# thomasneff/AdaNeRF

Measured on AMD Instinct MI355X. Metric: FPS at 800x800, higher is better.
Workload: dtype bf16

## Files before the change

adanerf_amd/csrc/k_mlp16.hip.hpp:

```cpp
#pragma once
#include "k_common.hip.hpp"
#include "k_mlp_f32.hip.hpp"
#include "tuning.hpp"
#include <utility>

namespace adanerf {


struct ShadeArgs {
  ShadeParams sp;
  NetParams net;
  const float* rays;
  const uint32_t* sample_key;
  const float* sample_z;
  const int32_t* total;
  int32_t max_samples;
  float* raw_out;
};

__device__ __forceinline__ void store_raw(const ShadeArgs& a, int s, float r, float g, float b, float alpha) {
  const float ks = a.net.out_scale[1];
  *reinterpret_cast<float4*>(a.raw_out + static_cast<size_t>(s) * 4) = make_float4(r * ks, g * ks, b * ks, alpha * a.net.out_scale[0]);
}

struct Bf16 {
  static constexpr bool kClampRelu = true;
  typedef bf16x8 vec8;
  static __device__ __forceinline__ uint32_t pack(float lo, float hi) {
    f32x2 v = {lo, hi};
    return __builtin_bit_cast(uint32_t, __builtin_convertvector(v, bf16x2));
  }
  static __device__ __forceinline__ f32x16 mfma(u32x4 a, u32x4 b, f32x16 c) {
    return __builtin_amdgcn_mfma_f32_32x32x16_bf16(__builtin_bit_cast(bf16x8, a), __builtin_bit_cast(bf16x8, b), c, 0, 0, 0);
  }
};
struct Fp16 {
  static constexpr bool kClampRelu = false;
  typedef f16x8 vec8;
  static __device__ __forceinline__ uint32_t pack(float lo, float hi) {
    f32x2 v = {lo, hi};
    return __builtin_bit_cast(uint32_t, __builtin_convertvector(v, f16x2));
  }
  static __device__ __forceinline__ f32x16 mfma(u32x4 a, u32x4 b, f32x16 c) {
    return __builtin_amdgcn_mfma_f32_32x32x16_f16(__builtin_bit_cast(f16x8, a), __builtin_bit_cast(f16x8, b), c, 0, 0, 0);
  }
};

using tune::kRegFrags;
constexpr int kShadeFrags16 = 32 + 4 * 128 + 160 + 2 * 128 + 144 + 72 + 8;
constexpr int kShadeBiasFloats = 8 * 256 + 288 + 128 + 32;

template <int CF, int RS, int LPW, int NR = kRegFrags>
struct WStream {
  static constexpr int kRegs = NR;
  static constexpr int kChunk = CF;
  static constexpr int kChunkBytes = CF * 1024;
#if defined(__HIP_DEVICE_COMPILE__)
  __amdgpu_buffer_rsrc_t rsrc;
#endif
  const char* gbase;
  uint32_t gbytes;
  uint32_t goff;
  uint32_t lane_off;
  uint32_t wave_off;
  uint32_t slot_cur;
  uint32_t rd_cur;
  uint32_t rd_next;
  uint32_t lds_base;
  uint32_t grp;
  uint32_t issuer;
  uint32_t dma_lds;
  uint32_t dma_goff;
  bool stag;
  u32x4 R[NR];
};

__device__ __forceinline__ u32x4 lds_read128(uint32_t byte_addr) {
  typedef const __attribute__((address_space(3))) u32x4* lds_u32x4_ptr;
  return *((lds_u32x4_ptr)(uintptr_t)byte_addr);
}

template <int CF, int RS, int LPW, int NR>
__device__ __forceinline__ void ws_piece(WStream<CF, RS, LPW, NR>& st, int i) {
  static_assert(LPW >= 1 && LPW <= 8, "a piece is addressed by the 12-bit immediate offset of buffer_load ... lds (pieces 4 .. 7: a second base)");
#if defined(__HIP_DEVICE_COMPILE__)
  typedef __attribute__((address_space(3))) void* lds_ptr;
  const uint32_t far = i >= 4 ? 4096u : 0u;
  lds_ptr dst = (lds_ptr) static_cast<uintptr_t>(st.dma_lds + far);
  const int voff = static_cast<int>(st.lane_off), soff = static_cast<int>(st.dma_goff + far);
  if (tune::kAblateDmaBytes) {
    if ((i & 3) == 0) __builtin_amdgcn_raw_ptr_buffer_load_lds(st.rsrc, dst, 4, voff, soff, 0, 0);
    else if ((i & 3) == 1) __builtin_amdgcn_raw_ptr_buffer_load_lds(st.rsrc, dst, 4, voff, soff, 1024, 0);
    else if ((i & 3) == 2) __builtin_amdgcn_raw_ptr_buffer_load_lds(st.rsrc, dst, 4, voff, soff, 2048, 0);
    else __builtin_amdgcn_raw_ptr_buffer_load_lds(st.rsrc, dst, 4, voff, soff, 3072, 0);
    return;
  }
  if ((i & 3) == 0) __builtin_amdgcn_raw_ptr_buffer_load_lds(st.rsrc, dst, 16, voff, soff, 0, 0);
  else if ((i & 3) == 1) __builtin_amdgcn_raw_ptr_buffer_load_lds(st.rsrc, dst, 16, voff, soff, 1024, 0);
  else if ((i & 3) == 2) __builtin_amdgcn_raw_ptr_buffer_load_lds(st.rsrc, dst, 16, voff, soff, 2048, 0);
  else __builtin_amdgcn_raw_ptr_buffer_load_lds(st.rsrc, dst, 16, voff, soff, 3072, 0);
#endif
}

template <int CF, int RS, int LPW, int NR>
__device__ __forceinline__ void ws_chunk_begin(WStream<CF, RS, LPW, NR>& st, uint32_t slot) {
  st.dma_lds = st.lds_base + slot * (CF * 1024) + st.wave_off;
  st.dma_goff = st.goff + st.wave_off;
  st.goff += CF * 1024;
  if (st.goff >= st.gbytes) st.goff = 0;
}

template <int CF, int RS, int LPW, int NR>
__device__ __forceinline__ void ws_issue(WStream<CF, RS, LPW, NR>& st, uint32_t slot) {
  ws_chunk_begin(st, slot);
#pragma unroll
  for (int i = 0; i < LPW; ++i) ws_piece(st, i);
}

__device__ __forceinline__ void ws_skip_pad() {
  if (tune::kSkipPad >= 0) asm volatile("s_nop %0" ::"n"(tune::kSkipPad < 0 ? 0 : tune::kSkipPad) : "memory");
}

template <int ABL, int CF, int RS, int LPW, int NR>
__device__ __forceinline__ void ws_sync(WStream<CF, RS, LPW, NR>& st, bool pad, int piece) {
  static_assert(RS >= 3 && (RS - 2) * LPW < 64, "vmcnt is a 6-bit counter");
  if (ABL & 1) return;
  if (!(ABL & 32)) asm volatile("s_waitcnt vmcnt(%0)\n\ts_barrier" ::"n"((RS - 3) * LPW) : "memory");
  const uint32_t slot = (st.grp == 0) ? st.slot_cur : (st.slot_cur == 0 ? RS - 1 : st.slot_cur - 1);
  if (!(ABL & 16)) {
    if (st.issuer) {
      ws_chunk_begin(st, slot);
      ws_piece(st, piece);
    } else if (pad) ws_skip_pad();
  }
}

template <int CF, int RS, int LPW, int NR>
__device__ __forceinline__ void ws_advance(WStream<CF, RS, LPW, NR>& st) {
  st.slot_cur = (st.slot_cur + 1 == RS) ? 0 : st.slot_cur + 1;
  const uint32_t nxt = (st.slot_cur + 1 == RS) ? 0 : st.slot_cur + 1;
  st.rd_cur = st.rd_next;
  st.rd_next = st.lds_base + nxt * (CF * 1024) + st.lane_off;
}


template <int ABL, int CF, int RS, int LPW, int NR>
__device__ __forceinline__ void ws_position(WStream<CF, RS, LPW, NR>& st, int f, bool tile_start) {
  constexpr int STEP = RS == 3 ? CF / LPW / 2 : CF / LPW;
  static_assert(CF % LPW == 0 && STEP >= 1 && (RS == 3 || (CF / 2) % STEP == 0), "piece positions: both groups' synchronisation points are piece positions");
  const bool pad = tile_start;
  const bool piece_pos = f % STEP == 0 && f / STEP < LPW && !(ABL & (1 | 16));
  if (f == 0) {
    if (ABL & 1) return;
    if (st.grp == 0) ws_sync<ABL>(st, pad, 0);
    else {
      if (pad) ws_skip_pad();
      if (piece_pos && st.issuer) ws_piece(st, 0);
    }
    ws_advance(st);
  } else if (f == CF / 2 && st.stag) {
    if (st.grp != 0) ws_sync<ABL>(st, pad, (CF / 2) / STEP);
    else {
      if (pad) ws_skip_pad();
      if (piece_pos && st.issuer) ws_piece(st, (CF / 2) / STEP);
    }
  } else if (piece_pos) {
    if (st.issuer) ws_piece(st, f / STEP);
  }
}

template <int ABL, int CF, int RS, int LPW, int NR>
__device__ __forceinline__ void ws_refill(WStream<CF, RS, LPW, NR>& st, int p) {
  if (ABL & 2) {
    asm volatile("" : "+v"(st.R[p % NR]));
    return;
  }
  const int q = p + NR;
  st.R[p % NR] = (q < CF) ? lds_read128(st.rd_cur + q * 1024) : lds_read128(st.rd_next + (q - CF) * 1024);
}

template <int CF, int RS, int LPW, int NR>
__device__ __forceinline__ void ws_start(WStream<CF, RS, LPW, NR>& st, const void* gbase, uint32_t gbytes, char* lds, int wave, int lane,
                                         int grp = -1, bool issuer = true) {
  st.stag = grp >= 0;
  st.grp = grp > 0 ? 1u : 0u;
  st.issuer = issuer;
  st.gbase = reinterpret_cast<const char*>(gbase);
  st.gbytes = gbytes;
#if defined(__HIP_DEVICE_COMPILE__)
  st.rsrc = __builtin_amdgcn_make_buffer_rsrc(const_cast<void*>(gbase), 0, static_cast<int>(gbytes), 0x00020000);
#endif
  st.goff = 0;
  st.lane_off = lane * 16;
  st.wave_off = wave * LPW * 1024;
  st.lds_base = static_cast<uint32_t>(reinterpret_cast<uintptr_t>(lds));
  if (issuer) {
#pragma unroll
    for (int k = 0; k < RS - 1; ++k) ws_issue(st, k);
  }
  asm volatile("s_waitcnt vmcnt(%0)\n\ts_barrier" ::"n"((RS - 2) * LPW) : "memory");
  st.slot_cur = RS - 1;
  st.rd_cur = st.lds_base + st.lane_off;
  st.rd_next = st.lds_base + st.lane_off;
#pragma unroll
  for (int i = 0; i < NR; ++i) st.R[i] = lds_read128(st.rd_next + i * 1024);
}

__device__ __forceinline__ float relu_keep_nan(float x) { return __builtin_elementwise_maximum(x, 0.0f); }

template <class ET, int F>
__device__ __forceinline__ void pe_pack(const float x[3], int h, uint32_t* out) {
  float t[pe_slots(F)];
  pe_eval<F, false>(x, h, t);
#pragma unroll
  for (int q = 0; q < pe_slots(F) / 2; ++q) out[q] = ET::pack(t[2 * q], t[2 * q + 1]);
}

struct BiasRegs {
  f32x4 b0, b1, b2, b3;
};
__device__ __forceinline__ void lds_bias_issue(uint32_t byte_addr, BiasRegs& r) {
  asm volatile("ds_read_b128 %0, %4\n\tds_read_b128 %1, %4 offset:16\n\tds_read_b128 %2, %4 offset:32\n\tds_read_b128 %3, %4 offset:48"
               : "=&v"(r.b0), "=&v"(r.b1), "=&v"(r.b2), "=&v"(r.b3)
               : "v"(byte_addr));
}
__device__ __forceinline__ void lds_bias_issue(uint32_t byte_addr, BiasRegs& r, uint32_t& rd0, uint32_t& rd1) {
  asm volatile("ds_read_b128 %0, %6\n\tds_read_b128 %1, %6 offset:16\n\tds_read_b128 %2, %6 offset:32\n\tds_read_b128 %3, %6 offset:48"
               : "=&v"(r.b0), "=&v"(r.b1), "=&v"(r.b2), "=&v"(r.b3), "+v"(rd0), "+v"(rd1)
               : "v"(byte_addr));
}
template <int YOUNGER = 0>
__device__ __forceinline__ void lds_bias_take(BiasRegs& r, f32x16* acc) {
  asm volatile("s_waitcnt lgkmcnt(%4)" : "+v"(r.b0), "+v"(r.b1), "+v"(r.b2), "+v"(r.b3) : "n"(YOUNGER > 15 ? 15 : YOUNGER));
  f32x16 a;
#pragma unroll
  for (int e = 0; e < 4; ++e) {
    a[e] = r.b0[e];
    a[4 + e] = r.b1[e];
    a[8 + e] = r.b2[e];
    a[12 + e] = r.b3[e];
  }
  *acc = a;
}

__device__ __forceinline__ void lds_bias16(uint32_t byte_addr, f32x16* acc) {
  f32x4 b0, b1, b2, b3;
  asm volatile("ds_read_b128 %0, %4\n\tds_read_b128 %1, %4 offset:16\n\tds_read_b128 %2, %4 offset:32\n\tds_read_b128 %3, %4 offset:48"
               : "=&v"(b0), "=&v"(b1), "=&v"(b2), "=&v"(b3)
               : "v"(byte_addr));
  asm volatile("s_waitcnt lgkmcnt(0)" : "+v"(b0), "+v"(b1), "+v"(b2), "+v"(b3));
  f32x16 a;
#pragma unroll
  for (int e = 0; e < 4; ++e) {
    a[e] = b0[e];
    a[4 + e] = b1[e];
    a[8 + e] = b2[e];
    a[12 + e] = b3[e];
  }
  *acc = a;
}

template <class ET, bool RELU>
__device__ __forceinline__ int mfma_guard(const f32x16& acc) {
  if constexpr (RELU && ET::kClampRelu) return __builtin_amdgcn_readfirstlane(__builtin_bit_cast(int, acc[15]));
  else return 0;
}

template <class ET, bool RELU>
__device__ __forceinline__ void epilogue_quad_16(const f32x16& acc, int m, int g, uint32_t* out, int guard = 0) {
  if constexpr (RELU && ET::kClampRelu) {
    uint32_t q0, q1;
    asm("v_cvt_pk_bf16_f32 %0, %1, %2 clamp\n\t; after the accumulator's guard %3" : "=v"(q0) : "v"(acc[4 * g + 0]), "v"(acc[4 * g + 1]), "s"(guard));
    asm("v_cvt_pk_bf16_f32 %0, %1, %2 clamp\n\t; after the accumulator's guard %3" : "=v"(q1) : "v"(acc[4 * g + 2]), "v"(acc[4 * g + 3]), "s"(guard));
    out[8 * m + 2 * g + 0] = q0;
    out[8 * m + 2 * g + 1] = q1;
    return;
  }
  uint32_t p0 = ET::pack(acc[4 * g + 0], acc[4 * g + 1]), p1 = ET::pack(acc[4 * g + 2], acc[4 * g + 3]);
  if (RELU) {
    if constexpr (std::is_same_v<ET, Fp16>) {
      const f16x2 z = {static_cast<_Float16>(0.f), static_cast<_Float16>(0.f)};
      p0 = __builtin_bit_cast(uint32_t, __builtin_elementwise_maximum(__builtin_bit_cast(f16x2, p0), z));
      p1 = __builtin_bit_cast(uint32_t, __builtin_elementwise_maximum(__builtin_bit_cast(f16x2, p1), z));
    } else {
      const s16x2 z = {0, 0};
      p0 = __builtin_bit_cast(uint32_t, __builtin_elementwise_max(__builtin_bit_cast(s16x2, p0), z));
      p1 = __builtin_bit_cast(uint32_t, __builtin_elementwise_max(__builtin_bit_cast(s16x2, p1), z));
    }
  }
  out[8 * m + 2 * g + 0] = p0;
  out[8 * m + 2 * g + 1] = p1;
}

constexpr int kKeepAllF32 = -2;


template <class ET, class WS, int S1, int S2, int MT, bool RELU, int FPOS, int KEEP_F32_TILE = -1>
__device__ __forceinline__ void layer_16(WS& st, uint32_t bias_addr, int lane, const uint32_t* in1, const uint32_t* in2,
                                         uint32_t* out, f32x16* keep = nullptr) {
  constexpr int CF = WS::kChunk;
  constexpr int KS = S1 + S2;
#pragma unroll
  for (int m = 0; m < MT; ++m) {
    f32x16 acc;
    if (tune::kAblateShade & 4) {
#pragma unroll
      for (int r = 0; r < 16; ++r) acc[r] = 0.f;
    } else {
      lds_bias16(bias_addr + m * 128, &acc);
    }
#pragma unroll
    for (int s = 0; s < KS; ++s) {
      const int f = (FPOS + m * KS + s) % CF;
      ws_position<tune::kAblateShade>(st, f, s == 0);
      const uint32_t* src = (s < S1) ? (in1 + 4 * s) : (in2 + 4 * (s - S1));
      u32x4 b = {src[0], src[1], src[2], src[3]};
      acc = ET::mfma(st.R[f % WS::kRegs], b, acc);
      ws_refill<tune::kAblateShade>(st, f);
    }
    if (KEEP_F32_TILE == kKeepAllF32) {
      keep[m] = acc;
    } else if (KEEP_F32_TILE == m) {
      *keep = acc;
    } else if (tune::kAblateShade & 8) {
      asm volatile("" ::"v"(acc));
#pragma unroll
      for (int g = 0; g < 8; ++g) asm volatile("" : "=v"(out[8 * m + g]));
    } else {
      const int gd = mfma_guard<ET, RELU>(acc);
#pragma unroll
      for (int g = 0; g < 4; ++g) epilogue_quad_16<ET, RELU>(acc, m, g, out, gd);
    }
  }
}

__device__ __forceinline__ void load_sample(const ShadeArgs& a, int s, int total, float x[3], float dpe[3]) {
  const int si = (s < total) ? s : (total > 0 ? total - 1 : 0);
  const uint32_t key = a.sample_key ? a.sample_key[si] : static_cast<uint32_t>(si);
  const uint32_t ray = key >> 7;
  const int bin = static_cast<int>(key & 127u);
  const float4* rr = reinterpret_cast<const float4*>(a.rays + static_cast<size_t>(ray) * 8);
  const float4 o4 = rr[0], d4 = rr[1];
  const float o[3] = {o4.x, o4.y, o4.z}, d[3] = {d4.x, d4.y, d4.z};
  sample_position(a.sp, o, d, a.sample_z ? a.sample_z[si] : a.sp.ztab[bin], x);
  if (a.sp.unit_dir) unit3(d, dpe);
  else {
    dpe[0] = d[0];
    dpe[1] = d[1];
    dpe[2] = d[2];
  }
}

template <int NQ>
__device__ __forceinline__ void lds_stash_write(uint32_t byte_addr, const uint32_t* v) {
#pragma unroll
  for (int g = 0; g < NQ; ++g) {
    const u32x4 t = {v[4 * g], v[4 * g + 1], v[4 * g + 2], v[4 * g + 3]};
    asm volatile("ds_write_b128 %0, %1" ::"v"(byte_addr + g * 1024), "v"(t) : "memory");
  }
}
template <int NQ>
__device__ __forceinline__ void lds_stash_read(uint32_t byte_addr, uint32_t* v) {
  u32x4 t[NQ];
#pragma unroll
  for (int g = 0; g < NQ; ++g) asm volatile("ds_read_b128 %0, %1" : "=&v"(t[g]) : "v"(byte_addr + g * 1024));
  if (NQ == 4) asm volatile("s_waitcnt lgkmcnt(0)" : "+v"(t[0]), "+v"(t[1]), "+v"(t[2]), "+v"(t[NQ > 3 ? 3 : 0]));
  else asm volatile("s_waitcnt lgkmcnt(0)" : "+v"(t[0]), "+v"(t[NQ > 1 ? 1 : 0]));
#pragma unroll
  for (int g = 0; g < NQ; ++g) {
    v[4 * g] = t[g][0];
    v[4 * g + 1] = t[g][1];
    v[4 * g + 2] = t[g][2];
    v[4 * g + 3] = t[g][3];
  }
}

template <class ET, int FP, int FD, int WAVES>
__global__ __launch_bounds__(WAVES * 64, WAVES == 8 ? 2 : 2) void shade_mlp16_kernel(ShadeArgs a) {
  static_assert(FP == 10 && FD == 4, "fragment positions below assume the 10-4 shading encoding");
  static_assert(WAVES == 4 || WAVES == 8, "chunk = 8 fragments");
  constexpr int QP = pe_slots(FP), QD = pe_slots(FD);
  constexpr bool kOneGroupDma = tune::kDmaGroup >= 0 && WAVES == 8;
  constexpr int TILE = WAVES * 32, CF = tune::kChunkFrags, RS = tune::kRingSlots, LPW = kOneGroupDma ? CF / 4 : CF / WAVES;
  constexpr int kRingBytes = CF * RS * 1024;
  static_assert(CF % WAVES == 0 && CF % kRegFrags == 0 && kShadeFrags16 % CF == 0 && CF % 8 == 0 && CF <= 32, "chunk geometry");
  typedef WStream<CF, RS, LPW> WS;
  constexpr int kStashBytes = WAVES * (QP / 8 + QD / 8) * 1024;
  __shared__ __attribute__((aligned(16))) char lds[kRingBytes + kShadeBiasFloats * 4 + kStashBytes];
  const int lane = lane_id();
  const int wave = __builtin_amdgcn_readfirstlane(static_cast<int>(threadIdx.x) >> 6);
  const int j = lane & 31, h = lane >> 5;
  const uint32_t stash = static_cast<uint32_t>(reinterpret_cast<uintptr_t>(lds)) + kRingBytes + kShadeBiasFloats * 4 +
                         wave * (QP / 8 + QD / 8) * 1024 + lane * 16;
  int total = a.total ? *a.total : a.max_samples;
  if (total > a.max_samples) total = a.max_samples;
  const int ntiles = (total + TILE - 1) / TILE;
  if (static_cast<int>(blockIdx.x) >= ntiles) return;

  {
    float* lds_bias = reinterpret_cast<float*>(lds + kRingBytes);
    for (int i = threadIdx.x; i < kShadeBiasFloats; i += blockDim.x) lds_bias[i] = a.net.bias[i];
  }
  __syncthreads();
  WS st;
  ws_start(st, a.net.w, kShadeFrags16 * 1024, lds, kOneGroupDma ? (wave & 3) : wave, lane,
           (tune::kStagger && WAVES == 8) ? (wave >> 2) : -1, !kOneGroupDma || (wave >> 2) == tune::kDmaGroup);

  const uint32_t bias0 = static_cast<uint32_t>(reinterpret_cast<uintptr_t>(lds)) + kRingBytes + h * 64;
  const uint32_t* bo = a.net.b_off;
  for (int tile = blockIdx.x; tile < ntiles; tile += gridDim.x) {
    const int s = tile * TILE + wave * 32 + j;
    uint32_t hA[64], hB[64];
    {
      float x[3], dpe[3];
      load_sample(a, s, total, x, dpe);
      uint32_t pts[QP / 2];
      pe_pack<ET, FP>(x, h, pts);
      uint32_t dirs[QD / 2];
      pe_pack<ET, FD>(dpe, h, dirs);
      lds_stash_write<QP / 8>(stash, pts);
      lds_stash_write<QD / 8>(stash + (QP / 8) * 1024, dirs);
      layer_16<ET, WS, QP / 8, 0, 8, true, 0>(st, bias0 + bo[0] * 4, lane, pts, pts, hA);
    }
#pragma unroll 1
    for (int l = 1; l <= 3; l += 2) {
      layer_16<ET, WS, 16, 0, 8, true, 0>(st, bias0 + bo[l] * 4, lane, hA, hA, hB);
      layer_16<ET, WS, 16, 0, 8, true, 0>(st, bias0 + bo[l + 1] * 4, lane, hB, hB, hA);
    }
    {
      uint32_t pts[QP / 2];
      lds_stash_read<QP / 8>(stash, pts);
      layer_16<ET, WS, QP / 8, 16, 8, true, 0>(st, bias0 + bo[5] * 4, lane, pts, hA, hB);
    }
    layer_16<ET, WS, 16, 0, 8, true, 0>(st, bias0 + bo[6] * 4, lane, hB, hB, hA);
    layer_16<ET, WS, 16, 0, 8, true, 0>(st, bias0 + bo[7] * 4, lane, hA, hA, hB);
    f32x16 alpha_tile;
    layer_16<ET, WS, 16, 0, 9, false, 0, 8>(st, bias0 + bo[8] * 4, lane, hB, hB, hA, &alpha_tile);
    const float alpha = alpha_tile[0];
    {
      uint32_t dirs[QD / 2];
      lds_stash_read<QD / 8>(stash + (QP / 8) * 1024, dirs);
      layer_16<ET, WS, 16, QD / 8, 4, true, (32 + 4 * 128 + 160 + 2 * 128 + 144) % CF>(st, bias0 + bo[9] * 4, lane, hA, dirs, hB);
    }
    f32x16 rgb_tile;
    layer_16<ET, WS, 8, 0, 1, false, (32 + 4 * 128 + 160 + 2 * 128 + 144 + 72) % CF, 0>(st, bias0 + bo[10] * 4, lane, hB, hB, hA, &rgb_tile);
    if (h == 0 && s < total)
      store_raw(a, s, rgb_tile[0], rgb_tile[1], rgb_tile[2], alpha);
  }
  asm volatile("s_waitcnt vmcnt(0)" ::: "memory");
}

struct PendingTile2 {
  f32x16 a, b;
};
template <class ET, class WS, int S1, int S2, int MT, bool RELU, int FPOS, int KEEP_F32_TILE = -1, int PEND_M = -1, bool PEND_RELU = true,
          bool CARRY_OUT = false>
__device__ __forceinline__ void layer_16x2(WS& st, uint32_t bias_addr, const uint32_t* in1A, const uint32_t* in2A, const uint32_t* in1B,
                                           const uint32_t* in2B, uint32_t* outA, uint32_t* outB, PendingTile2& pend, uint32_t* pendA = nullptr,
                                           uint32_t* pendB = nullptr, f32x16* keepA = nullptr, f32x16* keepB = nullptr) {
  constexpr int CF = WS::kChunk;
  constexpr int KS = S1 + S2;
  constexpr int ABL = tune::kAblateShade;
  constexpr int PER = (KS >= 8) ? 1 : (8 + KS - 1) / KS;
  constexpr bool kKeepAll = KEEP_F32_TILE == kKeepAllF32;
  auto kept = [](int m) { return kKeepAll || KEEP_F32_TILE == m; };
  constexpr bool kCarry = tune::kShadeCarry && !(ABL & 8);
  constexpr bool kHasPend = kCarry && PEND_M >= 0;
  constexpr int PERP = 1;
  static_assert(!kHasPend || KS >= 16, "a carried tile is consumed by the last two k-steps of a 16-k-step input segment, 6 k-steps behind its last conversion");
  static_assert(!CARRY_OUT || (KEEP_F32_TILE != MT - 1 && KEEP_F32_TILE != kKeepAllF32), "the kept tile is not converted");
  constexpr bool kCounted = tune::kBiasWaitCounted && tune::kSchedGroups && !(ABL & (2 | 4));
  constexpr int kYounger = kCounted ? KS : 0;
  BiasRegs br;
  f32x16 pA, pB;
  int gA = 0, gB = 0;
  if (kHasPend) {
    pA = pend.a;
    pB = pend.b;
  }
  if (!(ABL & 4)) lds_bias_issue(bias_addr, br, st.rd_cur, st.rd_next);
#pragma unroll
  for (int m = 0; m < MT; ++m) {
    f32x16 bias, accA, accB;
    if (tune::kSchedGroups) __builtin_amdgcn_sched_barrier(0);
    if (ABL & 4) {
#pragma unroll
      for (int r = 0; r < 16; ++r) bias[r] = 0.f;
    } else {
      if (m == 0) lds_bias_take<0>(br, &bias);
      else lds_bias_take<kYounger>(br, &bias);
      if (m + 1 < MT) lds_bias_issue(bias_addr + (m + 1) * 128, br, st.rd_cur, st.rd_next);
    }
#pragma unroll
    for (int s = 0; s < KS; ++s) {
      const int f = (FPOS + m * KS + s) % CF;
      ws_position<ABL>(st, f, false);
      const uint32_t* sa = (s < S1) ? (in1A + 4 * s) : (in2A + 4 * (s - S1));
      const uint32_t* sb = (s < S1) ? (in1B + 4 * s) : (in2B + 4 * (s - S1));
      const u32x4 ba = {sa[0], sa[1], sa[2], sa[3]}, bb = {sb[0], sb[1], sb[2], sb[3]};
      accA = ET::mfma(st.R[f % WS::kRegs], ba, s == 0 ? bias : accA);
      accB = ET::mfma(st.R[f % WS::kRegs], bb, s == 0 ? bias : accB);
      ws_refill<ABL>(st, f);
      constexpr int E0 = (tune::kShadeKstepFence && KS >= 8 + tune::kShadeGuardStep) ? tune::kShadeGuardStep : 0;
      if (m > 0 && !kept(m - 1) && !(ABL & 8) && s >= E0) {
        if (s == E0) {
          gA = mfma_guard<ET, RELU>(pA);
          gB = mfma_guard<ET, RELU>(pB);
        }
#pragma unroll
        for (int k = 0; k < PER; ++k) {
          const int q = (s - E0) * PER + k;
          if (q < 4) epilogue_quad_16<ET, RELU>(pA, m - 1, q, outA, gA);
          else if (q < 8) epilogue_quad_16<ET, RELU>(pB, m - 1, q - 4, outB, gB);
        }
      }
      if (m == 0 && kHasPend && s >= E0) {
        if (s == E0) {
          gA = mfma_guard<ET, PEND_RELU>(pA);
          gB = mfma_guard<ET, PEND_RELU>(pB);
        }
#pragma unroll
        for (int k = 0; k < PERP; ++k) {
          const int q = (s - E0) * PERP + k;
          if (q < 4) epilogue_quad_16<ET, PEND_RELU>(pA, PEND_M < 0 ? 0 : PEND_M, q, pendA, gA);
          else if (q < 8) epilogue_quad_16<ET, PEND_RELU>(pB, PEND_M < 0 ? 0 : PEND_M, q - 4, pendB, gB);
        }
      }
      if (tune::kSchedGroups) {
        __builtin_amdgcn_sched_group_barrier(0x008, 1, 0);
        __builtin_amdgcn_sched_group_barrier(0x002, 2, 0);
        __builtin_amdgcn_sched_group_barrier(0x008, 1, 0);
        __builtin_amdgcn_sched_group_barrier(0x100, 1, 0);
        __builtin_amdgcn_sched_group_barrier(0x002, 2, 0);
        if (tune::kShadeKstepFence) __builtin_amdgcn_sched_barrier(0);
      }
    }
    if (kept(m)) {
      keepA[kKeepAll ? m : 0] = accA;
      keepB[kKeepAll ? m : 0] = accB;
    }
    if ((ABL & 8) && !kept(m)) {
      asm volatile("" ::"v"(accA), "v"(accB));
#pragma unroll
      for (int g = 0; g < 8; ++g) asm volatile("" : "=v"(outA[8 * m + g]), "=v"(outB[8 * m + g]));
    } else if (m + 1 < MT) {
      pA = accA;
      pB = accB;
    } else if (!kept(m)) {
      if (CARRY_OUT && kCarry) {
        pend.a = accA;
        pend.b = accB;
      } else {
        gA = mfma_guard<ET, RELU>(accA);
        gB = mfma_guard<ET, RELU>(accB);
#pragma unroll
        for (int g = 0; g < 4; ++g) epilogue_quad_16<ET, RELU>(accA, m, g, outA, gA);
#pragma unroll
        for (int g = 0; g < 4; ++g) epilogue_quad_16<ET, RELU>(accB, m, g, outB, gB);
      }
    }
  }
}

template <class ET, int FP, int FD>
__global__ __launch_bounds__(256) void shade_mlp16x2_kernel(ShadeArgs a) {
  static_assert(FP == 10 && FD == 4, "fragment positions below assume the 10-4 shading encoding");
  constexpr int QP = pe_slots(FP), QD = pe_slots(FD);
  constexpr int WAVES = 4, TILE = WAVES * 64, CF = tune::kChunkFrags2, RS = tune::kRingSlots2, LPW = CF / WAVES;
  constexpr int kRingBytes = CF * RS * 1024;
  static_assert(CF % WAVES == 0 && CF % tune::kRegFrags2 == 0 && kShadeFrags16 % CF == 0 && CF % 8 == 0 && CF <= 32, "chunk geometry");
  typedef WStream<CF, RS, LPW, tune::kRegFrags2> WS;
  constexpr int kStashPerBlock = (QP / 8 + QD / 8) * 1024;
  __shared__ __attribute__((aligned(16))) char lds[kRingBytes + kShadeBiasFloats * 4 + WAVES * 2 * kStashPerBlock];
  const int lane = lane_id();
  const int wave = __builtin_amdgcn_readfirstlane(static_cast<int>(threadIdx.x) >> 6);
  const int j = lane & 31, h = lane >> 5;
  const uint32_t stash = static_cast<uint32_t>(reinterpret_cast<uintptr_t>(lds)) + kRingBytes + kShadeBiasFloats * 4 +
                         wave * 2 * kStashPerBlock + lane * 16;
  int total = a.total ? *a.total : a.max_samples;
  if (total > a.max_samples) total = a.max_samples;
  const int ntiles = (total + TILE - 1) / TILE;
  if (static_cast<int>(blockIdx.x) >= ntiles) return;
  {
    float* lds_bias = reinterpret_cast<float*>(lds + kRingBytes);
    for (int i = threadIdx.x; i < kShadeBiasFloats; i += blockDim.x) lds_bias[i] = a.net.bias[i];
  }
  __syncthreads();
  WS st;
  ws_start(st, a.net.w, kShadeFrags16 * 1024, lds, wave, lane);
  const uint32_t bias0 = static_cast<uint32_t>(reinterpret_cast<uintptr_t>(lds)) + kRingBytes + h * 64;
  const uint32_t* bo = a.net.b_off;
  for (int tile = blockIdx.x; tile < ntiles; tile += gridDim.x) {
    const int s0 = tile * TILE + wave * 64 + j, s1 = s0 + 32;
    uint32_t hA0[64], hB0[64], hA1[64], hB1[64];
    PendingTile2 pend;
    {
      float x[3], dpe[3];
      uint32_t pts0[QP / 2], pts1[QP / 2], dirs[QD / 2];
      load_sample(a, s0, total, x, dpe);
      pe_pack<ET, FP>(x, h, pts0);
      pe_pack<ET, FD>(dpe, h, dirs);
      lds_stash_write<QP / 8>(stash, pts0);
      lds_stash_write<QD / 8>(stash + (QP / 8) * 1024, dirs);
      load_sample(a, s1, total, x, dpe);
      pe_pack<ET, FP>(x, h, pts1);
      pe_pack<ET, FD>(dpe, h, dirs);
      lds_stash_write<QP / 8>(stash + kStashPerBlock, pts1);
      lds_stash_write<QD / 8>(stash + kStashPerBlock + (QP / 8) * 1024, dirs);
      layer_16x2<ET, WS, QP / 8, 0, 8, true, 0, -1, -1, true, true>(st, bias0 + bo[0] * 4, pts0, pts0, pts1, pts1, hA0, hA1, pend);
    }
#pragma unroll 1
    for (int l = 1; l <= 3; l += 2) {
      layer_16x2<ET, WS, 16, 0, 8, true, 0, -1, 7, true, true>(st, bias0 + bo[l] * 4, hA0, hA0, hA1, hA1, hB0, hB1, pend, hA0, hA1);
      layer_16x2<ET, WS, 16, 0, 8, true, 0, -1, 7, true, true>(st, bias0 + bo[l + 1] * 4, hB0, hB0, hB1, hB1, hA0, hA1, pend, hB0, hB1);
    }
    {
      uint32_t pts0[QP / 2], pts1[QP / 2];
      lds_stash_read<QP / 8>(stash, pts0);
      lds_stash_read<QP / 8>(stash + kStashPerBlock, pts1);
      layer_16x2<ET, WS, QP / 8, 16, 8, true, 0, -1, 7, true, true>(st, bias0 + bo[5] * 4, pts0, hA0, pts1, hA1, hB0, hB1, pend, hA0, hA1);
    }
    layer_16x2<ET, WS, 16, 0, 8, true, 0, -1, 7, true, true>(st, bias0 + bo[6] * 4, hB0, hB0, hB1, hB1, hA0, hA1, pend, hB0, hB1);
    layer_16x2<ET, WS, 16, 0, 8, true, 0, -1, 7, true, true>(st, bias0 + bo[7] * 4, hA0, hA0, hA1, hA1, hB0, hB1, pend, hA0, hA1);
    f32x16 alpha0, alpha1;
    layer_16x2<ET, WS, 16, 0, 9, false, 0, 8, 7, true, false>(st, bias0 + bo[8] * 4, hB0, hB0, hB1, hB1, hA0, hA1, pend, hB0, hB1, &alpha0, &alpha1);
    {
      uint32_t d0[QD / 2], d1[QD / 2];
      lds_stash_read<QD / 8>(stash + (QP / 8) * 1024, d0);
      lds_stash_read<QD / 8>(stash + kStashPerBlock + (QP / 8) * 1024, d1);
      layer_16x2<ET, WS, 16, QD / 8, 4, true, (32 + 4 * 128 + 160 + 2 * 128 + 144) % CF>(st, bias0 + bo[9] * 4, hA0, d0, hA1, d1, hB0, hB1, pend);
    }
    f32x16 rgb0, rgb1;
    layer_16x2<ET, WS, 8, 0, 1, false, (32 + 4 * 128 + 160 + 2 * 128 + 144 + 72) % CF, 0>(st, bias0 + bo[10] * 4, hB0, hB0, hB1, hB1, hA0, hA1, pend, nullptr, nullptr, &rgb0, &rgb1);
    if (h == 0 && s0 < total)
      store_raw(a, s0, rgb0[0], rgb0[1], rgb0[2], alpha0[0]);
    if (h == 0 && s1 < total)
      store_raw(a, s1, rgb1[0], rgb1[1], rgb1[2], alpha1[0]);
  }
  asm volatile("s_waitcnt vmcnt(0)" ::: "memory");
}

template <int FP, int FD>
__global__ __launch_bounds__(256) void shade_mlp32_kernel(ShadeArgs a) {
  constexpr int QP = pe_slots(FP), QD = pe_slots(FD);
  constexpr int TILE = 4 * 32;
  const int lane = lane_id();
  const int wave = __builtin_amdgcn_readfirstlane(static_cast<int>(threadIdx.x) >> 6);
  const int j = lane & 31, h = lane >> 5;
  int total = a.total ? *a.total : a.max_samples;
  if (total > a.max_samples) total = a.max_samples;
  const u32x4* w = a.net.w;
  const float* b = a.net.bias;

  for (int tile = blockIdx.x; tile * TILE < total; tile += gridDim.x) {
    const int s = tile * TILE + wave * 32 + j;
    if (tile * TILE + wave * 32 >= total) continue;
    asm volatile("" : "+v"(w), "+v"(b));
    float x[3], dpe[3];
    load_sample(a, s, total, x, dpe);
    float pts[QP], dirs[QD], hA[144], hB[128];
    pe_eval<FP, true>(x, h, pts);
    pe_eval<FD, true>(dpe, h, dirs);
    layer_f32<QP, 0, 8, true>(w + a.net.w_off[0], b + a.net.b_off[0], lane, pts, pts, hA);
#pragma unroll 1
    for (int l = 1; l <= 3; l += 2) {
      layer_f32<128, 0, 8, true>(w + a.net.w_off[l], b + a.net.b_off[l], lane, hA, hA, hB);
      layer_f32<128, 0, 8, true>(w + a.net.w_off[l + 1], b + a.net.b_off[l + 1], lane, hB, hB, hA);
    }
    layer_f32<QP, 128, 8, true>(w + a.net.w_off[5], b + a.net.b_off[5], lane, pts, hA, hB);
    layer_f32<128, 0, 8, true>(w + a.net.w_off[6], b + a.net.b_off[6], lane, hB, hB, hA);
    layer_f32<128, 0, 8, true>(w + a.net.w_off[7], b + a.net.b_off[7], lane, hA, hA, hB);
    layer_f32<128, 0, 9, false>(w + a.net.w_off[8], b + a.net.b_off[8], lane, hB, hB, hA);
    const float alpha = hA[128];
    layer_f32<128, QD, 4, true>(w + a.net.w_off[9], b + a.net.b_off[9], lane, hA, dirs, hB);
    float rgb[16];
    layer_f32<64, 0, 1, false>(w + a.net.w_off[10], b + a.net.b_off[10], lane, hB, hB, rgb);
    if (h == 0 && s < total)
      *reinterpret_cast<float4*>(a.raw_out + static_cast<size_t>(s) * 4) = make_float4(rgb[0], rgb[1], rgb[2], alpha);
  }
}

static __global__ __launch_bounds__(256) void shade_features_kernel(ShadeArgs a, float* feat, int FP, int FD) {
  const int s = blockIdx.x * blockDim.x + threadIdx.x;
  if (s >= a.max_samples) return;
  float x[3], dpe[3];
  load_sample(a, s, a.max_samples, x, dpe);
  const int NP = 3 + 6 * FP, ND = 3 + 6 * FD;
  float* f = feat + static_cast<size_t>(s) * (NP + ND);
  for (int c = 0; c < 3; ++c) {
    f[c] = x[c];
    f[NP + c] = dpe[c];
  }
  for (int b = 0; b < FP; ++b)
    for (int c = 0; c < 3; ++c) {
      float sn, co;
      sincosf(x[c] * static_cast<float>(1 << b), &sn, &co);
      f[3 + 6 * b + c] = sn;
      f[3 + 6 * b + 3 + c] = co;
    }
  for (int b = 0; b < FD; ++b)
    for (int c = 0; c < 3; ++c) {
      float sn, co;
      sincosf(dpe[c] * static_cast<float>(1 << b), &sn, &co);
      f[NP + 3 + 6 * b + c] = sn;
      f[NP + 3 + 6 * b + 3 + c] = co;
    }
}

}
```

adanerf_amd/csrc/tuning.hpp:

```cpp
#pragma once

namespace adanerf {
namespace tune {

constexpr int kChunkFrags = 16, kRingSlots = 4;
constexpr int kRegFrags = 4;
constexpr bool kStagger = true;
constexpr int kDmaGroup = 0;
constexpr int kSkipPad = 11;
constexpr int kShadeBlocks = 2;
constexpr bool kFastPeFp16Pass = true;
constexpr bool kSchedGroups = true, kSchedGroupsSampling = true;
constexpr int kSgbValuSampling = 4;
constexpr bool kBiasWaitCounted = true, kSplitBiasCounted = true;
constexpr bool kShadeCarry = true, kSplitCarry = true;
constexpr bool kShadeKstepFence = true, kSplitKstepFence = true;
constexpr int kShadeGuardStep = 2;
constexpr bool kGenericStaged = true;
constexpr int kGenericBlocks128 = 2, kGenericBlocks256 = 2;
constexpr int kGenericOcc64 = 2, kGenericOcc128 = 2, kGenericOcc256 = 1;
constexpr int kGenericBlocks512 = 1, kGenericOcc512 = 1;
constexpr int kGenericSpread = 1;
constexpr bool kGenericBiasDirect = true;
constexpr int kGenericAhead = 4;
constexpr int kSelRaysPerBlock = 64;

#if !defined(ADN_EXPERIMENT) && (defined(ADN_CF_S) || defined(ADN_RS_S) || defined(ADN_NR_S) || defined(ADN_CF2) || defined(ADN_RS2) || defined(ADN_NR2) || \
                                 defined(ADN_ABLATE) || defined(ADN_ABLATE_S) || defined(ADN_ABLATE_G) || defined(ADN_ABLATE_DMA_BYTES))
#error "ADN_<NAME> overrides are for experiment builds: add -DADN_EXPERIMENT (tools/ablate.sh does)"
#endif
#ifndef ADN_CF_S
#define ADN_CF_S 32
#endif
#ifndef ADN_RS_S
#define ADN_RS_S 3
#endif
#ifndef ADN_NR_S
#define ADN_NR_S 16
#endif
#ifndef ADN_CF2
#define ADN_CF2 32
#endif
#ifndef ADN_RS2
#define ADN_RS2 3
#endif
#ifndef ADN_NR2
#define ADN_NR2 16
#endif
constexpr int kChunkFragsSampling = ADN_CF_S, kRingSlotsSampling = ADN_RS_S, kRegFragsSampling = ADN_NR_S;
constexpr int kChunkFrags2 = ADN_CF2, kRingSlots2 = ADN_RS2, kRegFrags2 = ADN_NR2;

#ifndef ADN_ABLATE
#define ADN_ABLATE 0
#endif
#ifndef ADN_ABLATE_S
#define ADN_ABLATE_S 0
#endif
#ifndef ADN_ABLATE_G
#define ADN_ABLATE_G 0
#endif
#ifndef ADN_ABLATE_DMA_BYTES
#define ADN_ABLATE_DMA_BYTES 0
#endif
constexpr int kAblateShade = ADN_ABLATE, kAblateSample = ADN_ABLATE_S, kAblateGeneric = ADN_ABLATE_G;
constexpr bool kAblateDmaBytes = ADN_ABLATE_DMA_BYTES != 0;

}
}
```

Before: 226.6.

## Prefetch next tile's sample keys and ray records into LDS during shading layers

Adds a software prefetch for the persistent shading kernel. During layer 0 it issues global-to-LDS loads of the next tile's sample keys and z values, and during the skip layer it reads those keys and issues global-to-LDS loads of the ray records. The next tile then reads its inputs from LDS instead of doing dependent global gathers at the start of each tile. This costs extra LDS, inline asm that juggles M0, and a blocking lgkmcnt wait inside the MFMA loop. The ray records reuse the position stash area, which is a correctness risk.

```diff
diff --git a/adanerf_amd/csrc/k_mlp16.hip.hpp b/adanerf_amd/csrc/k_mlp16.hip.hpp
--- a/adanerf_amd/csrc/k_mlp16.hip.hpp
+++ b/adanerf_amd/csrc/k_mlp16.hip.hpp
@@ -334,15 +334,19 @@
   }
 }
 
+__device__ __forceinline__ void sample_inputs(const ShadeArgs& a, float4 o4, float4 d4, float z, float x[3], float dpe[3]);
 __device__ __forceinline__ void load_sample(const ShadeArgs& a, int s, int total, float x[3], float dpe[3]) {
   const int si = (s < total) ? s : (total > 0 ? total - 1 : 0);
   const uint32_t key = a.sample_key ? a.sample_key[si] : static_cast<uint32_t>(si);
   const uint32_t ray = key >> 7;
   const int bin = static_cast<int>(key & 127u);
   const float4* rr = reinterpret_cast<const float4*>(a.rays + static_cast<size_t>(ray) * 8);
-  const float4 o4 = rr[0], d4 = rr[1];
+  sample_inputs(a, rr[0], rr[1], a.sample_z ? a.sample_z[si] : a.sp.ztab[bin], x, dpe);
+}
+
+__device__ __forceinline__ void sample_inputs(const ShadeArgs& a, float4 o4, float4 d4, float z, float x[3], float dpe[3]) {
   const float o[3] = {o4.x, o4.y, o4.z}, d[3] = {d4.x, d4.y, d4.z};
-  sample_position(a.sp, o, d, a.sample_z ? a.sample_z[si] : a.sp.ztab[bin], x);
+  sample_position(a.sp, o, d, z, x);
   if (a.sp.unit_dir) unit3(d, dpe);
   else {
     dpe[0] = d[0];
@@ -453,11 +457,14 @@
 struct PendingTile2 {
   f32x16 a, b;
 };
+struct NoFill {
+  __device__ __forceinline__ void step(int, int) {}
+};
 template <class ET, class WS, int S1, int S2, int MT, bool RELU, int FPOS, int KEEP_F32_TILE = -1, int PEND_M = -1, bool PEND_RELU = true,
-          bool CARRY_OUT = false>
+          bool CARRY_OUT = false, class FILL = NoFill>
 __device__ __forceinline__ void layer_16x2(WS& st, uint32_t bias_addr, const uint32_t* in1A, const uint32_t* in2A, const uint32_t* in1B,
                                            const uint32_t* in2B, uint32_t* outA, uint32_t* outB, PendingTile2& pend, uint32_t* pendA = nullptr,
-                                           uint32_t* pendB = nullptr, f32x16* keepA = nullptr, f32x16* keepB = nullptr) {
+                                           uint32_t* pendB = nullptr, f32x16* keepA = nullptr, f32x16* keepB = nullptr, FILL* fill = nullptr) {
   constexpr int CF = WS::kChunk;
   constexpr int KS = S1 + S2;
   constexpr int ABL = tune::kAblateShade;
@@ -501,6 +508,7 @@
       accA = ET::mfma(st.R[f % WS::kRegs], ba, s == 0 ? bias : accA);
       accB = ET::mfma(st.R[f % WS::kRegs], bb, s == 0 ? bias : accB);
       ws_refill<ABL>(st, f);
+      if (fill) fill->step(m, s);
       constexpr int E0 = (tune::kShadeKstepFence && KS >= 8 + tune::kShadeGuardStep) ? tune::kShadeGuardStep : 0;
       if (m > 0 && !kept(m - 1) && !(ABL & 8) && s >= E0) {
         if (s == E0) {
@@ -562,6 +570,62 @@
   }
 }
 
+template <int BYTES>
+__device__ __forceinline__ void glds_copy(const void* src, uint32_t lds_dst) {
+  uint32_t keep;
+  if constexpr (BYTES == 16)
+    asm volatile("s_mov_b32 %0, m0\n\ts_mov_b32 m0, %2\n\ts_nop 0\n\tglobal_load_lds_dwordx4 %1, off\n\ts_mov_b32 m0, %0\n\ts_nop 0"
+                 : "=&s"(keep) : "v"(src), "s"(lds_dst) : "memory");
+  else
+    asm volatile("s_mov_b32 %0, m0\n\ts_mov_b32 m0, %2\n\ts_nop 0\n\tglobal_load_lds_dword %1, off\n\ts_mov_b32 m0, %0\n\ts_nop 0"
+                 : "=&s"(keep) : "v"(src), "s"(lds_dst) : "memory");
+}
+
+struct ShadePrefetch {
+  const ShadeArgs* a;
+  int total, lane;
+  int next;
+  uint32_t rec;
+  uint32_t kz;
+  __device__ __forceinline__ int sample_index() const {
+    const int n = next + lane;
+    return n < total ? n : total - 1;
+  }
+};
+struct PrefetchKeys : ShadePrefetch {
+  __device__ __forceinline__ void step(int m, int s) {
+    if (m != 0 || s != 1) return;
+    const int si = sample_index();
+    const void* dummy = a->net.bias + lane;
+    glds_copy<4>(a->sample_key ? static_cast<const void*>(a->sample_key + si) : dummy, kz);
+    glds_copy<4>(a->sample_z ? static_cast<const void*>(a->sample_z + si) : dummy, kz + 256);
+  }
+};
+struct PrefetchRecords : ShadePrefetch {
+  __device__ __forceinline__ void step(int m, int s) {
+    if (m != 0 || s != 1) return;
+    uint32_t key;
+    asm volatile("ds_read_b32 %0, %1\n\ts_waitcnt lgkmcnt(0)" : "=&v"(key) : "v"(kz + lane * 4) : "memory");
+    if (!a->sample_key) key = static_cast<uint32_t>(sample_index());
+    const float* rr = a->rays + static_cast<size_t>(key >> 7) * 8;
+    glds_copy<16>(rr, rec);
+    glds_copy<16>(rr + 4, rec + 1024);
+  }
+};
+__device__ __forceinline__ void load_sample_prefetched(const ShadeArgs& a, const ShadePrefetch& pf, int s, int idx, float x[3], float dpe[3]) {
+  f32x4 o4, d4;
+  uint32_t key;
+  float z;
+  asm volatile("ds_read_b128 %0, %4\n\tds_read_b128 %1, %4 offset:1024\n\tds_read_b32 %2, %5\n\tds_read_b32 %3, %5 offset:256\n\ts_waitcnt lgkmcnt(0)"
+               : "=&v"(o4), "=&v"(d4), "=&v"(key), "=&v"(z)
+               : "v"(pf.rec + idx * 16), "v"(pf.kz + idx * 4)
+               : "memory");
+  const int si = s < pf.total ? s : pf.total - 1;
+  if (!a.sample_key) key = static_cast<uint32_t>(si);
+  if (!a.sample_z) z = a.sp.ztab[key & 127u];
+  sample_inputs(a, make_float4(o4[0], o4[1], o4[2], o4[3]), make_float4(d4[0], d4[1], d4[2], d4[3]), z, x, dpe);
+}
+
 template <class ET, int FP, int FD>
 __global__ __launch_bounds__(256) void shade_mlp16x2_kernel(ShadeArgs a) {
   static_assert(FP == 10 && FD == 4, "fragment positions below assume the 10-4 shading encoding");
@@ -571,12 +635,14 @@
   static_assert(CF % WAVES == 0 && CF % tune::kRegFrags2 == 0 && kShadeFrags16 % CF == 0 && CF % 8 == 0 && CF <= 32, "chunk geometry");
   typedef WStream<CF, RS, LPW, tune::kRegFrags2> WS;
   constexpr int kStashPerBlock = (QP / 8 + QD / 8) * 1024;
-  __shared__ __attribute__((aligned(16))) char lds[kRingBytes + kShadeBiasFloats * 4 + WAVES * 2 * kStashPerBlock];
+  constexpr bool kPrefetch = tune::kShadePrefetch;
+  static_assert((QP / 8) * 1024 >= 2048, "the ray records take the block-0 position stash");
+  __shared__ __attribute__((aligned(16))) char lds[kRingBytes + kShadeBiasFloats * 4 + WAVES * 2 * kStashPerBlock + (kPrefetch ? WAVES * 512 : 0)];
   const int lane = lane_id();
   const int wave = __builtin_amdgcn_readfirstlane(static_cast<int>(threadIdx.x) >> 6);
   const int j = lane & 31, h = lane >> 5;
-  const uint32_t stash = static_cast<uint32_t>(reinterpret_cast<uintptr_t>(lds)) + kRingBytes + kShadeBiasFloats * 4 +
-                         wave * 2 * kStashPerBlock + lane * 16;
+  const uint32_t stash_wave = static_cast<uint32_t>(reinterpret_cast<uintptr_t>(lds)) + kRingBytes + kShadeBiasFloats * 4 + wave * 2 * kStashPerBlock;
+  const uint32_t stash = stash_wave + lane * 16;
   int total = a.total ? *a.total : a.max_samples;
   if (total > a.max_samples) total = a.max_samples;
   const int ntiles = (total + TILE - 1) / TILE;
@@ -590,24 +656,37 @@
   ws_start(st, a.net.w, kShadeFrags16 * 1024, lds, wave, lane);
   const uint32_t bias0 = static_cast<uint32_t>(reinterpret_cast<uintptr_t>(lds)) + kRingBytes + h * 64;
   const uint32_t* bo = a.net.b_off;
+  ShadePrefetch pf;
+  pf.a = &a;
+  pf.total = total;
+  pf.lane = lane;
+  pf.rec = stash_wave;
+  pf.kz = static_cast<uint32_t>(reinterpret_cast<uintptr_t>(lds)) + kRingBytes + kShadeBiasFloats * 4 + WAVES * 2 * kStashPerBlock + wave * 512;
   for (int tile = blockIdx.x; tile < ntiles; tile += gridDim.x) {
     const int s0 = tile * TILE + wave * 64 + j, s1 = s0 + 32;
     uint32_t hA0[64], hB0[64], hA1[64], hB1[64];
     PendingTile2 pend;
+    const bool fetched = kPrefetch && tile != static_cast<int>(blockIdx.x);
+    pf.next = (tile + gridDim.x) * TILE + wave * 64;
     {
       float x[3], dpe[3];
       uint32_t pts0[QP / 2], pts1[QP / 2], dirs[QD / 2];
-      load_sample(a, s0, total, x, dpe);
+      if (fetched) load_sample_prefetched(a, pf, s0, j, x, dpe);
+      else load_sample(a, s0, total, x, dpe);
       pe_pack<ET, FP>(x, h, pts0);
       pe_pack<ET, FD>(dpe, h, dirs);
+      if (fetched) load_sample_prefetched(a, pf, s1, 32 + j, x, dpe);
       lds_stash_write<QP / 8>(stash, pts0);
       lds_stash_write<QD / 8>(stash + (QP / 8) * 1024, dirs);
-      load_sample(a, s1, total, x, dpe);
+      if (!fetched) load_sample(a, s1, total, x, dpe);
       pe_pack<ET, FP>(x, h, pts1);
       pe_pack<ET, FD>(dpe, h, dirs);
       lds_stash_write<QP / 8>(stash + kStashPerBlock, pts1);
       lds_stash_write<QD / 8>(stash + kStashPerBlock + (QP / 8) * 1024, dirs);
-      layer_16x2<ET, WS, QP / 8, 0, 8, true, 0, -1, -1, true, true>(st, bias0 + bo[0] * 4, pts0, pts0, pts1, pts1, hA0, hA1, pend);
+      PrefetchKeys fk;
+      static_cast<ShadePrefetch&>(fk) = pf;
+      layer_16x2<ET, WS, QP / 8, 0, 8, true, 0, -1, -1, true, true>(st, bias0 + bo[0] * 4, pts0, pts0, pts1, pts1, hA0, hA1, pend, nullptr, nullptr,
+                                                                    nullptr, nullptr, kPrefetch ? &fk : nullptr);
     }
 #pragma unroll 1
     for (int l = 1; l <= 3; l += 2) {
@@ -618,7 +697,10 @@
       uint32_t pts0[QP / 2], pts1[QP / 2];
       lds_stash_read<QP / 8>(stash, pts0);
       lds_stash_read<QP / 8>(stash + kStashPerBlock, pts1);
-      layer_16x2<ET, WS, QP / 8, 16, 8, true, 0, -1, 7, true, true>(st, bias0 + bo[5] * 4, pts0, hA0, pts1, hA1, hB0, hB1, pend, hA0, hA1);
+      PrefetchRecords fr;
+      static_cast<ShadePrefetch&>(fr) = pf;
+      layer_16x2<ET, WS, QP / 8, 16, 8, true, 0, -1, 7, true, true>(st, bias0 + bo[5] * 4, pts0, hA0, pts1, hA1, hB0, hB1, pend, hA0, hA1, nullptr, nullptr,
+                                                                     kPrefetch ? &fr : nullptr);
     }
     layer_16x2<ET, WS, 16, 0, 8, true, 0, -1, 7, true, true>(st, bias0 + bo[6] * 4, hB0, hB0, hB1, hB1, hA0, hA1, pend, hB0, hB1);
     layer_16x2<ET, WS, 16, 0, 8, true, 0, -1, 7, true, true>(st, bias0 + bo[7] * 4, hA0, hA0, hA1, hA1, hB0, hB1, pend, hA0, hA1);
diff --git a/adanerf_amd/csrc/tuning.hpp b/adanerf_amd/csrc/tuning.hpp
--- a/adanerf_amd/csrc/tuning.hpp
+++ b/adanerf_amd/csrc/tuning.hpp
@@ -26,7 +26,8 @@
 constexpr int kSelRaysPerBlock = 64;
 
 #if !defined(ADN_EXPERIMENT) && (defined(ADN_CF_S) || defined(ADN_RS_S) || defined(ADN_NR_S) || defined(ADN_CF2) || defined(ADN_RS2) || defined(ADN_NR2) || \
-                                 defined(ADN_ABLATE) || defined(ADN_ABLATE_S) || defined(ADN_ABLATE_G) || defined(ADN_ABLATE_DMA_BYTES))
+                                 defined(ADN_ABLATE) || defined(ADN_ABLATE_S) || defined(ADN_ABLATE_G) || defined(ADN_ABLATE_DMA_BYTES) || \
+                                 defined(ADN_SHADE_PREFETCH))
 #error "ADN_<NAME> overrides are for experiment builds: add -DADN_EXPERIMENT (tools/ablate.sh does)"
 #endif
 #ifndef ADN_CF_S
@@ -49,6 +50,10 @@
 #endif
 constexpr int kChunkFragsSampling = ADN_CF_S, kRingSlotsSampling = ADN_RS_S, kRegFragsSampling = ADN_NR_S;
 constexpr int kChunkFrags2 = ADN_CF2, kRingSlots2 = ADN_RS2, kRegFrags2 = ADN_NR2;
+#ifndef ADN_SHADE_PREFETCH
+#define ADN_SHADE_PREFETCH 1
+#endif
+constexpr bool kShadePrefetch = ADN_SHADE_PREFETCH != 0;
 
 #ifndef ADN_ABLATE
 #define ADN_ABLATE 0
```

Result: no change. 226.9, median of 6 (+0.1%).
